# ugadiarov-la-phystech-edu/OCRL

Measured on AMD Instinct MI355X. Metric: images/sec (node) SLATE pretrain 128x128, 6 slots, 3 iters, higher is better.
Workload: dtype f32

## Files before the change

ocrl_amd/_lib.py:

```python
import ctypes
import os
from ctypes import c_void_p

from . import _abi

_HERE = os.path.dirname(os.path.abspath(__file__))
LIB_PATH = os.environ.get("OCRL_HIP_LIB") or os.path.join(_HERE, "libocrl_hip.so")
HEADER_PATH = os.path.join(_HERE, os.pardir, "include", "ocrl_hip.h")
DQN_HEADER_PATH = os.path.join(_HERE, os.pardir, "include", "ocrl_hip_dqn.h")
ROLLOUT_HEADER_PATH = os.path.join(_HERE, os.pardir, "include", "ocrl_hip_rollout.h")
REPLAY_HEADER_PATH = os.path.join(_HERE, os.pardir, "include", "ocrl_hip_replay.h")
C51_HEADER_PATH = os.path.join(_HERE, os.pardir, "include", "ocrl_hip_c51.h")
_lib = None

if not os.path.exists(HEADER_PATH):
    raise RuntimeError(f"{HEADER_PATH} is missing: ocrl_amd derives its binding of libocrl_hip.so from the header and runs from the source tree.")
with open(HEADER_PATH) as _f:
    ABI = _abi.read(_f.read())
CONSTANTS = ABI.consts
SlateConfig, IodineConfig, GemmDesc, ConvDesc, ConvWgradDesc, XattnDesc, AcnetDesc, SpriteEnvDesc, ScenesDesc, FlatSegment = (
    ABI.structs["ocrl_" + n] for n in ("slate_config", "iodine_config", "gemm_desc", "conv_desc", "conv_wgrad_desc", "xattn_desc", "acnet_desc",
                                       "sprite_env_desc", "scenes_desc", "flat_segment"))
FLAT_MAX_SEGMENTS = CONSTANTS["OCRL_FLAT_MAX_SEGMENTS"]
if not os.path.exists(DQN_HEADER_PATH):
    raise RuntimeError(f"{DQN_HEADER_PATH} is missing: ocrl_amd derives its binding of libocrl_hip.so from the header and runs from the source tree.")
with open(DQN_HEADER_PATH) as _f:
    ABI_DQN = _abi.read(_f.read())
QnetDesc = ABI_DQN.structs["ocrl_qnet_desc"]
QNET_MAX_LAYERS = len(QnetDesc().dims)
if not os.path.exists(ROLLOUT_HEADER_PATH):
    raise RuntimeError(f"{ROLLOUT_HEADER_PATH} is missing: ocrl_amd derives its binding of libocrl_hip.so from the header and runs from the source tree.")
with open(ROLLOUT_HEADER_PATH) as _f:
    ABI_ROLLOUT = _abi.read(_f.read())
if not os.path.exists(REPLAY_HEADER_PATH):
    raise RuntimeError(f"{REPLAY_HEADER_PATH} is missing: ocrl_amd derives its binding of libocrl_hip.so from the header and runs from the source tree.")
with open(REPLAY_HEADER_PATH) as _f:
    ABI_REPLAY = _abi.read(_f.read())
if not os.path.exists(C51_HEADER_PATH):
    raise RuntimeError(f"{C51_HEADER_PATH} is missing: ocrl_amd derives its binding of libocrl_hip.so from the header and runs from the source tree.")
with open(C51_HEADER_PATH) as _f:
    ABI_C51 = _abi.read(_f.read())
C51Desc = ABI_C51.structs["ocrl_c51_desc"]


def flat_segments(segs):
    addr = lambda a: a.value if isinstance(a, c_void_p) else a
    return (FlatSegment * len(segs))(*[FlatSegment(addr(p), addr(g), addr(s0), addr(s1), int(n)) for p, g, s0, s1, n in segs])


def acnet_desc(B, F, A, dims, acts):
    d = AcnetDesc(B=B, F=F, A=A)
    for t in range(3):
        if len(dims[t]) > CONSTANTS["OCRL_ACNET_MAX_LAYERS"]:
            raise ValueError(f"ocrl_amd: at most {CONSTANTS['OCRL_ACNET_MAX_LAYERS']} layers per trunk (got {len(dims[t])})")
        d.n[t] = len(dims[t])
        for l, (w, a) in enumerate(zip(dims[t], acts[t])):
            d.dims[t][l], d.acts[t][l] = int(w), int(a)
    return d


def qnet_desc(B, F, A, dims, acts):
    if len(dims) > QNET_MAX_LAYERS or len(acts) != len(dims):
        raise ValueError(f"ocrl_amd: at most {QNET_MAX_LAYERS} hidden layers, one activation code each (got {len(dims)}, {len(acts)})")
    d = QnetDesc(B=B, F=F, A=A, n=len(dims))
    for l, (w, a) in enumerate(zip(dims, acts)):
# ... 21 lines not shown
    d = ConvDesc()
    for k, v in kw.items():
        setattr(d, k, v)
    return d


def conv_wgrad_desc(**kw):
    d = ConvWgradDesc()
    for k, v in kw.items():
        setattr(d, k, v)
    return d


def lib():
    global _lib
    if _lib is not None:
        return _lib
    if not os.path.exists(LIB_PATH):
        raise RuntimeError(
            f"{LIB_PATH} is missing: build it with `python -c 'import __graft_entry__ as g; g.build()'` "
            "(make -C ocrl_amd/csrc).  ocrl_amd has no CPU fallback.")
    import torch
    L = ctypes.CDLL(LIB_PATH)
    for abi in (ABI, ABI_DQN, ABI_ROLLOUT, ABI_REPLAY, ABI_C51):
        for name, (restype, argtypes) in abi.functions.items():
            f = getattr(L, name)
            f.argtypes = argtypes
            if restype is not ctypes.c_int:
                f.restype = restype
    for name, cls in {**ABI.structs, **ABI_DQN.structs, **ABI_C51.structs}.items():
        if name + "_size" in {**ABI.functions, **ABI_DQN.functions, **ABI_C51.functions} and getattr(L, name + "_size")() != ctypes.sizeof(cls):
            raise RuntimeError(f"libocrl_hip.so: {name} is {getattr(L, name + '_size')()} bytes, this binding's {cls.__name__} {ctypes.sizeof(cls)}")
    if L.ocrl_abi_version() != CONSTANTS["OCRL_ABI_VERSION"]:
        raise RuntimeError(f"libocrl_hip.so ABI version mismatch: the library is {L.ocrl_abi_version()}, include/ocrl_hip.h {CONSTANTS['OCRL_ABI_VERSION']}")
    _lib = L
    return L


def check(rc):
    if rc:
        raise RuntimeError("ocrl_hip: " + lib().ocrl_last_error().decode())


def ptr(t):
    return None if t is None else ctypes.c_void_p(t.data_ptr())


# ... 8 lines not shown
```

ocrl_amd/csrc/kernels.h:

```cpp
#pragma once
#include "common.h"
#include "../../include/ocrl_hip.h"

enum { PROF_CONV5 = 0, PROF_CONV_OTHER = 1, PROF_WGRAD = 2, PROF_GEMM = 3, PROF_SA_FWD = 4, PROF_SA_BWD = 5, PROF_ATTN_FWD = 6, PROF_ATTN_BWD = 7, PROF_NTAGS = 8 };
int prof_begin(int tag, hipStream_t st);
void prof_end(int idx, hipStream_t st);

struct GemmArgs {
    const float* A = nullptr;
    const float* B = nullptr;
    float* C = nullptr;
    int M = 0, N = 0, K = 0;
    int lda = 0, ldb = 0, ldc = 0;
    int akc = 1, bkc = 1;
    int batch = 1;
    int batch_inner = 1;
    long long sA = 0, sB = 0, sC = 0;
    long long sAi = 0, sBi = 0, sCi = 0;
    int splitk = 1;
    long long sCsplit = 0;
    float alpha = 1.f;
    const float* bias = nullptr;
    int relu = 0;
    float drop_p = 0.f;
// ... 190 lines not shown
    int B = 0, H = 0, W = 0;
    float* bpart = nullptr;
};
int conv_fwd_launch(const ConvArgs& a, int KS, int CIN, int COUT, hipStream_t st, int low_latency = 0);
int conv_wgrad_launch(const WgradArgs& a, int KS, int CIN, int COUT, int cin_real, float* dW, float* db, int accumulate, hipStream_t st, int x3 = -1);
int conv_wgrad_slabs(int B, int H, int W, int KS, int CIN);
size_t conv_wgrad_ws_floats(int B, int H, int W, int KS, int CIN, bool with_db = true);
int conv_pack_launch(const float* W, float* fwd, float* bwd, int KS, int CIN, int COUT, int cin_real, hipStream_t st);

size_t conv_first_pack_floats();
int conv_first_pack_launch(const float* W, float* pack, hipStream_t st);
int conv_first_fwd_launch(const float* obs, const float* pack, const float* bias, float* Y, int B, int H, int W, int relu, hipStream_t st);
int conv_first_wgrad_workers(int B, int H, int W);
size_t conv_first_wgrad_ws_floats(int B, int H, int W);
int conv_first_wgrad_launch(const float* obs, const float* dY, float* ws, float* dW, float* db, int B, int H, int W, int accumulate, hipStream_t st);

int nchw_to_nhwc8_launch(const float* in, float* out, int B, int C, int H, int W, hipStream_t st);
int patchify4_launch(const float* in, float* out, int B, int C, int S, hipStream_t st);
int pixel_shuffle_launch(const float* in, float* out, int B, int h, int w, int Cout, int forward, const float* mask, hipStream_t st);
int layernorm_fwd_launch(const float* x, const float* g, const float* b, float* y, float* mean, float* rstd, long long R, int F, hipStream_t st);
int layernorm_bwd_launch(const float* dy, const float* x, const float* mean, const float* rstd, const float* g, float* dx,
                         float* dgb, long long R, int F, int accumulate_dx, int accumulate_dgb, float* ws, size_t ws_floats, hipStream_t st);
int colsum_launch(const float* X, long long ld, float* out, long long R, int F, int accumulate, float scale, float* ws, size_t ws_floats, hipStream_t st);

#define SA_INPUT_SLAB (2 * 4096 + 4 * 64)
void sa_input_plan(long long R, int max_wgs, int out[3]);
int sa_input_fwd_launch(const float* e4, const float* gamma, const float* beta, const float* W0, const float* b0, const float* W2, const float* b2,
                        float* mean, float* rstd, float* ln0, float* h1, float* x, long long R, int max_wgs, hipStream_t st);
int sa_input_bwd_launch(const float* dx, const float* h1, const float* e4, const float* mean, const float* rstd, const float* gamma, const float* beta,
                        const float* W0, const float* W2, float* de4, float* dW0, float* db0, float* dW2, float* db2, float* dgamma, float* dbeta,
                        long long R, int max_wgs, float* ws, size_t ws_floats, hipStream_t st);
int reduce_partials_launch(const float* part, int n, float* out, float scale, int accumulate, hipStream_t st);
int mse_launch(const float* obs, const float* recon, float* drecon, float* out, int B, int C, int H, int W, float* ws, size_t ws_floats, hipStream_t st);
int gumbel_softmax_launch(const float* raw, const float* e1, const float* e2, float* z, int* tokens, long long R, int V, float tau,
                          unsigned long long seed, hipStream_t st, float* zst = nullptr);
int softmax_bwd_rows_launch(const float* z, float* d, long long R, int V, float scale, hipStream_t st);
int softmax_stat_combine_launch(const float* stat, int nseg, long long R, float* lse, const float* hstat, const int* hidx, int* tokens,
                                const float* pred, int ldp, const int* tok, float* out, float scale, float* ws, size_t ws_floats, hipStream_t st,
                                const float* cdf_scores = nullptr, int cdf_V = 0, float cdf_tau = 1.f, unsigned long long cdf_seed = 0);
int exp_rows_launch(const float* y, const float* lse, float* z, long long R, int V, hipStream_t st);
int rowdot_bias64_launch(const float* g, const float* act, const float* bias, long long R, float* out, hipStream_t st);
int embed_fwd_launch(const int* tokens, const float* dict, const float* bos, const float* pe, float* out, int B, int T, int d, float p,
                     unsigned long long seed, hipStream_t st);
size_t embed_bwd_ws_floats(long long BT, int V, int d);
int embed_bwd_launch(float* g, const int* tokens, float* ddict, int B, int T, int V, int d, float p, unsigned long long seed, float* ws,
                     size_t ws_floats, hipStream_t st);
// ... 211 lines not shown
```

ocrl_amd/csrc/slate_model.cpp:

```cpp
#include "slate_model.h"

#include "switches.h"

#include <math.h>
#include <stdarg.h>
#include <string.h>

static std::string fmt(const char* f, ...) {
    char buf[256];
    va_list ap;
    va_start(ap, f);
    vsnprintf(buf, sizeof buf, f, ap);
    va_end(ap);
    return buf;
}

SlateModel::SlateModel(const SlateConfig& c) : cfg(c) {
    S = c.obs_size; E = S / 4; T = E * E; N = S * S; V = c.vocab; d = c.d_model; C = c.cnn_hidden;
    K = c.num_slots; I = c.num_iters; D = c.slot_size; H = c.mlp_hidden; NB = c.num_blocks; NH = c.num_heads;
    DH = d / NH; Bmax = c.max_batch; SH = c.slot_heads > 0 ? c.slot_heads : 1;
    const int ch = c.obs_channels;
    add_param("_dvae._encoder.0.m.weight", {64, ch, 4, 4}, 0); add_param("_dvae._encoder.0.m.bias", {64}, 0);
    for (int i = 1; i < 7; ++i) { add_param(fmt("_dvae._encoder.%d.m.weight", i), {64, 64, 1, 1}, 0); add_param(fmt("_dvae._encoder.%d.m.bias", i), {64}, 0); }
    add_param("_dvae._encoder.7.weight", {V, 64, 1, 1}, 0); add_param("_dvae._encoder.7.bias", {V}, 0);
// ... 165 lines not shown
                if (ws_commit_) { x3_of_[bc_pk_[i]] = f3; x3_of_[bc_pkb_[i]] = b3; }
            }
        }
        bc_Wk4_ = carve(nullptr, 9 * 64 * 4); bc_Wb4_ = carve(nullptr, 9 * 64 * 4);
        bc_dW1r_ = carve(nullptr, (size_t)25 * 64 * D); bc_dWc_ = carve(nullptr, 25 * 64 * 5 + 64);
        bc_dT_ = carve(nullptr, BK * 1600); bc_dM_ = carve(nullptr, BK * 1600); bc_G1_ = carve(nullptr, (size_t)N * 64);
        recon_ = carve("recon", BN * 4);
    } else {
    patches_ = carve("patches", BT * 16 * cfg.obs_channels);
    for (int i = 0; i < 7; ++i) de_[i] = carve(fmt("dvae_enc%d", i).c_str(), BT * 64);
    zraw_ = carve("zraw", BT * V);
    z_ = carve("z", BT * V);
    zdec_ = cfg.hard ? carve("z_st", BT * V) : z_;
    tokens_ = reinterpret_cast<int*>(carve("tokens", BT));
    {
        const size_t nseg = (size_t)gemm_stat_segments(V);
        zstat_ = carve(nullptr, BT * nseg * 2); zhstat_ = carve(nullptr, BT * nseg); zhidx_ = reinterpret_cast<int*>(carve(nullptr, BT * nseg));
        zlse_ = carve("z_lse", BT); zdot_ = carve(nullptr, BT);
        cestat_ = carve(nullptr, BT * nseg * 2); celse_ = carve("ce_lse", BT); cepart_ = carve(nullptr, BT / 16 + 16);
    }
    dd0_ = carve("dvae_dec0", BT * 64); dd1_ = carve("dvae_dec1", BT * 64); dd2_ = carve("dvae_dec2", BT * 64); dd3_ = carve("dvae_dec3", BT * 64);
    dd4_ = carve("dvae_dec4", BT * 256); ps1_ = carve(nullptr, BT * 256);
    dd6_ = carve("dvae_dec6", BT * 256); dd7_ = carve("dvae_dec7", BT * 256); dd8_ = carve("dvae_dec8", BT * 256);
    dd9_ = carve("dvae_dec9", BT * 1024); ps2_ = carve(nullptr, BN * 64);
    recon_ = carve("recon", BN * 4); drecon_ = carve(nullptr, BN * 4);
    for (int i = 0; i < 2; ++i) {
        dw_fwd_[i] = carve(nullptr, 9 * 64 * 64); dw_bwd_[i] = carve(nullptr, 9 * 64 * 64);
        if (conv_x3_ > 0) {
            float* f3 = carve(nullptr, conv_x3_pack_floats(3));
            float* b3 = carve(nullptr, conv_x3_pack_floats(3));
            if (ws_commit_) { x3_of_[dw_fwd_[i]] = f3; x3_of_[dw_bwd_[i]] = b3; }
        }
    }
    w11p_ = carve(nullptr, 4 * 64);
    mem_ = carve("mem", BK * d); emb_ = carve("emb", BT * d);
    for (int b = 0; b < NB; ++b) {
        Blk& k = blk_[b];
        k.ln1 = carve(nullptr, BT * d); k.ln1_mean = carve(nullptr, BT); k.ln1_rstd = carve(nullptr, BT);
        k.q = carve(nullptr, BT * 3 * d); k.k = k.q + d; k.v = k.q + 2 * d;
        k.lse = carve(nullptr, B * NH * (size_t)T); k.ao = carve(nullptr, BT * d); k.x1 = carve(nullptr, BT * d);
        k.ln2 = carve(nullptr, BT * d); k.ln2_mean = carve(nullptr, BT); k.ln2_rstd = carve(nullptr, BT);
        k.cq = carve(nullptr, BT * d); k.ck = carve(nullptr, BK * d); k.cv = carve(nullptr, BK * d);
        k.cP = carve(nullptr, B * NH * (size_t)T * K); k.cao = carve(nullptr, BT * d); k.x2 = carve(nullptr, BT * d);
        k.ln3 = carve(nullptr, BT * d); k.ln3_mean = carve(nullptr, BT); k.ln3_rstd = carve(nullptr, BT);
        k.f1 = carve(fmt("blk%d.ffn_hidden", b).c_str(), BT * 4 * d); k.x3 = carve(nullptr, BT * d);
    }
    bg_.resize(NB);
    {
        const size_t NC = xattn_supported(K, d, NH) ? (size_t)NH * xattn_kp(K, NH) : 16;
        xa_zero_base_ = carve_pos();
        for (int b = 0; b < NB; ++b) {
            Blk& k = blk_[b];
            k.xaAb = carve(nullptr, B * NC * d); k.xaAbT = carve(nullptr, B * NC * d); k.xaVo = carve(nullptr, B * NC * d); k.xaVoT = carve(nullptr, B * NC * d);
        }
        xa_zero_floats_ = (size_t)(carve_pos() - xa_zero_base_);
        for (int b = 0; b < NB; ++b) { bg_[b].xaPd = carve(nullptr, BT * NC); bg_[b].xaDs = carve(nullptr, BT * NC); }
        xa_dAb_ = carve(nullptr, B * NC * d); xa_dVo_ = carve(nullptr, B * NC * d);
// ... 93 lines not shown
}

int SlateModel::pack_weights(const Lane& L, bool encoder_only) {
    if (first_direct()) RC(conv_first_pack_launch(P(w_.enc[0].w), cw_fwd_[0], L));
    else RC(conv_pack_launch(P(w_.enc[0].w), cw_fwd_[0], nullptr, 5, 8, 64, cfg.obs_channels, L));
    RC(conv_pack_launch(P(w_.enc[1].w), cw_fwd_[1], cw_bwd_[1], 5, 64, 64, 64, L));
    RC(conv_pack_launch(P(w_.enc[2].w), cw_fwd_[2], cw_bwd_[2], 5, 64, 64, 64, L));
    RC(conv_pack_launch(P(w_.enc[3].w), cw_fwd_[3], cw_bwd_[3], 5, 64, 64, 64, L));
    if (conv_x3_ > 0) {
        for (int i = 1; i < 4; ++i) {
            auto f = x3_of_.find(cw_fwd_[i]), b = x3_of_.find(cw_bwd_[i]);
            if (f != x3_of_.end()) RC(conv_pack_x3_launch(P(w_.enc[i].w), const_cast<float*>(f->second), b != x3_of_.end() ? const_cast<float*>(b->second) : nullptr, L));
        }
    }
    if (!cfg.use_bcdec && !encoder_only) {
        RC(conv_pack_launch(P(w_.dvae_dec[1].w), dw_fwd_[0], dw_bwd_[0], 3, 64, 64, 64, L));
        RC(conv_pack_launch(P(w_.dvae_dec[6].w), dw_fwd_[1], dw_bwd_[1], 3, 64, 64, 64, L));
        if (conv_x3_ > 0) {
            for (int i = 0; i < 2; ++i) {
                auto f = x3_of_.find(dw_fwd_[i]), b = x3_of_.find(dw_bwd_[i]);
                if (f != x3_of_.end()) RC(conv_pack_x3_launch(P(w_.dvae_dec[i ? 6 : 1].w), const_cast<float*>(f->second), b != x3_of_.end() ? const_cast<float*>(b->second) : nullptr, L, 3));
            }
        }
        RC(copy_launch(P(w_.dvae_dec[11].w), w11p_, cfg.obs_channels * 64, L));
        RC(fill_launch(w11p_ + cfg.obs_channels * 64, (4 - cfg.obs_channels) * 64, 0.f, L));
    }
    RC(pack_launch(sa_pack_dev_, sa_pack_n_, sa_pack_max_, sa_wts_, L));
    RC(posmap_launch(P(w_.enc_pos.w), P(w_.enc_pos.b), posmap_, S, C, L));
    return 0;
}

int SlateModel::fwd_encoder(const StepInputs& in, const Lane& L, FwdDvae fork) {
    const int B = in.B;
    const long long BN = (long long)B * N;
    auto fork_if = [&](FwdDvae here) -> int {
        if (fork != here) return 0;
        RC(after(dvae_lane(), L, ev_fork_));
        return fwd_dvae(in, dvae_lane());
    };
    RC(slot_init_launch(P(w_.sa.mu), P(w_.sa.log_sigma), in.noise_slots, slots0_, B * K, D, in.seed, L, in.seed_dev));
    SlotAttnArgs a = sa_args(B, N, K, D, H, I, SH);
    a.x = x_; a.slots0 = slots0_; a.wts = sa_wts_; a.slots = slots_; a.attn = attn_; a.attn_heads = attn_heads_; a.save = sa_save_;
    if (conv_lowlat_ && frozen_) a.save = nullptr;
    a.xchg = sa_xchg_; a.parts = sa_parts_;
    a.phase = 1;
    RC(slot_attn_launch(a, 0, L));
    RC(fork_if(FwdDvae::AtStart));
    if (first_direct()) {
// ... 51 lines not shown
}

int SlateModel::dvae_decode(int B, float* drecon, const Lane& L, const float* zin) {
    const long long BT = (long long)B * T, BN = (long long)B * N;
    const int ch = cfg.obs_channels;
    if (!zin && fused_heads()) {
        GemmArgs a;
        a.A = zraw_; a.B = P(w_.dvae_dec[0].w); a.C = dd0_; a.M = (int)BT; a.N = 64; a.K = V; a.lda = V; a.ldb = V; a.ldc = 64;
        a.bias = P(w_.dvae_dec[0].b); a.relu = 1; a.a_mode = 2; a.x_lse = zlse_;
        RC(gemm_launch(a, L));
    } else {
    if (!zin) zin = zdec_;
    RC(lin_fwd(zin, V, P(w_.dvae_dec[0].w), P(w_.dvae_dec[0].b), dd0_, 64, BT, 64, V, 1, nullptr, 0, 0.f, 0, L));
    }
    RC(conv_layer_fwd(dd0_, dw_fwd_[0], P(w_.dvae_dec[1].b), dd1_, B, E, E, 3, 64, 1, nullptr, nullptr, L));
    RC(lin_fwd(dd1_, 64, P(w_.dvae_dec[2].w), P(w_.dvae_dec[2].b), dd2_, 64, BT, 64, 64, 1, nullptr, 0, 0.f, 0, L));
    RC(lin_fwd(dd2_, 64, P(w_.dvae_dec[3].w), P(w_.dvae_dec[3].b), dd3_, 64, BT, 64, 64, 1, nullptr, 0, 0.f, 0, L));
    RC(lin_fwd(dd3_, 64, P(w_.dvae_dec[4].w), P(w_.dvae_dec[4].b), dd4_, 256, BT, 256, 64, 1, nullptr, 0, 0.f, 0, L));
    RC(pixel_shuffle_launch(dd4_, ps1_, B, E, E, 64, 1, nullptr, L));
    RC(conv_layer_fwd(ps1_, dw_fwd_[1], P(w_.dvae_dec[6].b), dd6_, B, 2 * E, 2 * E, 3, 64, 1, nullptr, nullptr, L));
    RC(lin_fwd(dd6_, 64, P(w_.dvae_dec[7].w), P(w_.dvae_dec[7].b), dd7_, 64, 4 * BT, 64, 64, 1, nullptr, 0, 0.f, 0, L));
    RC(lin_fwd(dd7_, 64, P(w_.dvae_dec[8].w), P(w_.dvae_dec[8].b), dd8_, 64, 4 * BT, 64, 64, 1, nullptr, 0, 0.f, 0, L));
    RC(lin_fwd(dd8_, 64, P(w_.dvae_dec[9].w), P(w_.dvae_dec[9].b), dd9_, 256, 4 * BT, 256, 64, 1, nullptr, 0, 0.f, 0, L));
    RC(pixel_shuffle_launch(dd9_, ps2_, B, 2 * E, 2 * E, 64, 1, nullptr, L));
    RC(lin_fwd(ps2_, 64, P(w_.dvae_dec[11].w), P(w_.dvae_dec[11].b), recon_, 4, BN, ch, 64, 0, nullptr, 0, 0.f, 0, L));
    RC(mse_launch(last_.obs, recon_, drecon, metrics_ + (drecon ? 0 : 4), B, ch, S, S, L.scratch, L.scratch_floats, L));
    return 0;
}

AttnArgs SlateModel::self_attn_args(int b) const {
    const Blk& k = blk_[b];
    AttnArgs a;
    a.q = k.q; a.k = k.k; a.v = k.v; a.o = k.ao; a.lse = k.lse; a.B = last_.B; a.T = T; a.d = d; a.h = NH; a.ld = 3 * d;
    a.p = pdrop_; a.seed = last_.seed; a.site = SITE_BLK_BASE + 8 * b + 0;
    return a;
}
XaHost SlateModel::xattn_args(int b) const {
    const Blk& k = blk_[b];
    const unsigned site = SITE_BLK_BASE + 8 * b;
    XaHost hx;
    hx.x = k.ln2; hx.P = k.cP; hx.Ab = k.xaAb; hx.AbT = k.xaAbT; hx.Vo = k.xaVo; hx.VoT = k.xaVoT;
    hx.B = last_.B; hx.T = T; hx.K = K; hx.d = d; hx.h = NH; hx.p = pdrop_; hx.seed = last_.seed; hx.site_p = site + 2; hx.site_o = site + 3;
    return hx;
}

int SlateModel::fwd_decoder(const Lane& L, bool with_ce) {
    const int B = last_.B;
    const long long BT = (long long)B * T;
// ... 349 lines not shown
    RC(colsum_launch(gmap_, C, G(w_.enc[3].b), N, C, 0, 1.f, L.scratch, L.scratch_floats, L));
    RC(conv_layer_wgrad(e3_, gB_, G(w_.enc[3].w), nullptr, B, S, S, 5, 64, 64, L));
    RC(conv_layer_fwd(gB_, cw_bwd_[3], nullptr, gA_, B, S, S, 5, 64, 0, nullptr, e3_, L));
    RC(conv_layer_wgrad(e2_, gA_, G(w_.enc[2].w), G(w_.enc[2].b), B, S, S, 5, 64, 64, L));
    RC(conv_layer_fwd(gA_, cw_bwd_[2], nullptr, gB_, B, S, S, 5, 64, 0, nullptr, e2_, L));
    RC(conv_layer_wgrad(e1_, gB_, G(w_.enc[1].w), G(w_.enc[1].b), B, S, S, 5, 64, 64, L));
    RC(conv_layer_fwd(gB_, cw_bwd_[1], nullptr, gA_, B, S, S, 5, 64, 0, nullptr, e1_, L));
    if (first_direct()) {
        OCRL_REQUIRE(conv_first_wgrad_ws_floats(B, S, S) <= L.scratch_floats, "first conv wgrad: scratch too small");
        RC(conv_first_wgrad_launch(obs_keep_, gA_, L.scratch, G(w_.enc[0].w), G(w_.enc[0].b), B, S, S, 0, L));
    } else {
        const int ch = cfg.obs_channels, ldc0 = (25 * ch + 3) & ~3;
        if (!side_w) RC(im2col5_launch(obs8_, col0_, BN, S, S, ch, ldc0, L));
        RC(lin_bwd_w(gA_, 64, col0_, ldc0, dw0p_, G(w_.enc[0].b), BN, 64, ldc0, 1.f, L));
        RC(unpack5_launch(dw0p_, G(w_.enc[0].w), ch, ldc0, L));
    }
    return 0;
}

int SlateModel::bwd_dvae(const Lane& L) {
    const int B = last_.B;
    const long long BT = (long long)B * T, BN = (long long)B * N;
    const int ch = cfg.obs_channels;
    float* w4 = L.scratch + L.scratch_floats - 1024;
    {
        GemmArgs a;
        a.A = drecon_; a.B = ps2_; a.C = w4; a.M = 4; a.N = 64; a.K = (int)BN; a.lda = 4; a.ldb = 64; a.ldc = 64; a.akc = 0; a.bkc = 0;
        long long splits = BN / 512; if (splits > 512) splits = 512; if (splits < 1) splits = 1;
        if (splits > 1) {
            a.splitk = (int)splits; a.C = L.scratch; a.sCsplit = 256;
            RC(gemm_launch(a, L));
            RC(splitk_reduce_launch(L.scratch, w4, 256, (int)splits, 256, 0, L));
        } else RC(gemm_launch(a, L));
        RC(copy_launch(w4, G(w_.dvae_dec[11].w), ch * 64, L));
        RC(colsum_launch(drecon_, 4, w4 + 256, BN, 4, 0, 1.f, L.scratch, L.scratch_floats - 1024, L));
        RC(copy_launch(w4 + 256, G(w_.dvae_dec[11].b), ch, L));
    }
    RC(lin_bwd_x(drecon_, 4, w11p_, gdA_, 64, BN, 4, 64, nullptr, 0, nullptr, 0, L));
    RC(pixel_shuffle_launch(gdA_, gdB_, B, 2 * E, 2 * E, 64, 0, dd9_, L));
    RC(lin_bwd_w(gdB_, 256, dd8_, 64, G(w_.dvae_dec[9].w), G(w_.dvae_dec[9].b), 4 * BT, 256, 64, 1.f, L));
    RC(lin_bwd_x(gdB_, 256, P(w_.dvae_dec[9].w), gdA_, 64, 4 * BT, 256, 64, dd8_, 64, nullptr, 0, L));
    RC(lin_bwd_w(gdA_, 64, dd7_, 64, G(w_.dvae_dec[8].w), G(w_.dvae_dec[8].b), 4 * BT, 64, 64, 1.f, L));
    RC(lin_bwd_x(gdA_, 64, P(w_.dvae_dec[8].w), gdB_, 64, 4 * BT, 64, 64, dd7_, 64, nullptr, 0, L));
    RC(lin_bwd_w(gdB_, 64, dd6_, 64, G(w_.dvae_dec[7].w), G(w_.dvae_dec[7].b), 4 * BT, 64, 64, 1.f, L));
    RC(lin_bwd_x(gdB_, 64, P(w_.dvae_dec[7].w), gdA_, 64, 4 * BT, 64, 64, dd6_, 64, nullptr, 0, L));
    RC(conv_layer_wgrad(ps1_, gdA_, G(w_.dvae_dec[6].w), G(w_.dvae_dec[6].b), B, 2 * E, 2 * E, 3, 64, 64, L));
    RC(conv_layer_fwd(gdA_, dw_bwd_[1], nullptr, gdB_, B, 2 * E, 2 * E, 3, 64, 0, nullptr, ps1_, L));
    RC(pixel_shuffle_launch(gdB_, gdA_, B, E, E, 64, 0, nullptr, L));
    RC(lin_bwd_w(gdA_, 256, dd3_, 64, G(w_.dvae_dec[4].w), G(w_.dvae_dec[4].b), BT, 256, 64, 1.f, L));
    RC(lin_bwd_x(gdA_, 256, P(w_.dvae_dec[4].w), gdB_, 64, BT, 256, 64, dd3_, 64, nullptr, 0, L));
    RC(lin_bwd_w(gdB_, 64, dd2_, 64, G(w_.dvae_dec[3].w), G(w_.dvae_dec[3].b), BT, 64, 64, 1.f, L));
    RC(lin_bwd_x(gdB_, 64, P(w_.dvae_dec[3].w), gdA_, 64, BT, 64, 64, dd2_, 64, nullptr, 0, L));
    RC(lin_bwd_w(gdA_, 64, dd1_, 64, G(w_.dvae_dec[2].w), G(w_.dvae_dec[2].b), BT, 64, 64, 1.f, L));
    RC(lin_bwd_x(gdA_, 64, P(w_.dvae_dec[2].w), gdB_, 64, BT, 64, 64, dd1_, 64, nullptr, 0, L));
    RC(conv_layer_wgrad(dd0_, gdB_, G(w_.dvae_dec[1].w), G(w_.dvae_dec[1].b), B, E, E, 3, 64, 64, L));
    RC(conv_layer_fwd(gdB_, dw_bwd_[0], nullptr, gdA_, B, E, E, 3, 64, 0, nullptr, dd0_, L));
    float* dz = zraw_;
    have_scores_ = false;
    if (fused_heads()) {
        Xf zx; zx.b_mode = 2; zx.lse = zlse_;
        RC(lin_bwd_w(gdA_, 64, zraw_, V, G(w_.dvae_dec[0].w), G(w_.dvae_dec[0].b), BT, 64, V, 1.f, L, zx));
        RC(rowdot_bias64_launch(gdA_, dd0_, P(w_.dvae_dec[0].b), BT, zdot_, L));
// ... 128 lines not shown
```

ocrl_amd/csrc/slate_model.h:

```cpp
#pragma once
#include <map>
#include <string>
#include <vector>

#include "kernels.h"
#include "model_base.h"
#include "slot_attn_host.h"
#include "stream_plan.h"

struct SlateConfig {
    int obs_size = 64, obs_channels = 3, vocab = 4096, d_model = 192, cnn_hidden = 64;
    int num_slots = 5, num_iters = 3, slot_size = 192, mlp_hidden = 192;
    int num_blocks = 4, num_heads = 4;
    float dropout = 0.1f;
    int max_batch = 1;
    int use_bcdec = 0;
    int hard = 0;
    int slot_heads = 1;
};

struct StepInputs {
    const float* obs = nullptr;
    int B = 0;
    float tau = 1.f;
// ... 87 lines not shown
    long long group_begin_[4] = {0, 0, 0, 0};

    int S, E, T, N, V, d, C, K, I, D, H, NB, NH, DH, Bmax;
    int SH = 1;
    StepInputs last_;
    float pdrop_ = 0.f;
    bool have_fwd_ = false;
    int conv_lowlat_ = 0;
    bool frozen_ = false, packs_valid_ = false;
    bool have_enc_ = false;
    bool enc_only_grads_ = false;
    bool have_scores_ = false;

    float *scratch_ = nullptr;
    size_t scratch_floats_ = 0;
    float* scratch2_ = nullptr;
    StreamPlan plan_;
    hipStream_t side_ = nullptr;
    hipEvent_t ev_fork_ = nullptr, ev_join_ = nullptr, ev_tokens_ = nullptr;
    float *zstat_ = nullptr, *zhstat_ = nullptr, *zlse_ = nullptr, *zdot_ = nullptr, *cestat_ = nullptr, *celse_ = nullptr, *cepart_ = nullptr;
    int* zhidx_ = nullptr;
    float *obs8_, *patches_, *de_[7], *zraw_, *z_, *zdec_;
    int* tokens_;
    float *dd0_, *dd1_, *dd2_, *dd3_, *dd4_, *ps1_, *dd6_, *dd7_, *dd8_, *dd9_, *ps2_, *recon_, *drecon_;
    float *e1_, *e2_, *e3_, *e4_, *posmap_, *gridT_, *ln0_, *ln0_mean_, *ln0_rstd_, *h1_, *x_;
    float *slots0_, *slot_noise_, *slots_, *attn_, *sa_save_, *sa_wts_, *sa_grows_, *sa_small_, *sa_xchg_;
    float* attn_heads_ = nullptr;
    float* sa_parts_;
    PackEntry* sa_pack_dev_ = nullptr;
    int sa_pack_n_ = 0, sa_pack_max_ = 0;
    float *cw_fwd_[4], *cw_bwd_[4];
    int conv_x3_ = 0;
    std::map<const float*, const float*> x3_of_;
    float *dw_fwd_[2], *dw_bwd_[2];
    float *w11p_;
    float *mem_, *emb_;
    struct Blk {
        float *ln1, *ln1_mean, *ln1_rstd, *q, *k, *v, *lse, *ao, *x1;
        float *ln2, *ln2_mean, *ln2_rstd, *cq, *ck, *cv, *cP, *cao, *x2;
        float *ln3, *ln3_mean, *ln3_rstd, *f1, *x3;
        float *xaAb, *xaAbT, *xaVo, *xaVoT;
    };
    int sa_input_ = 1;
    bool xattn_ = false;
    float *xa_dAb_ = nullptr, *xa_dVo_ = nullptr, *xa_pq_ = nullptr, *xa_po_ = nullptr;
    size_t xa_zero_floats_ = 0;
    float* xa_zero_base_ = nullptr;
    std::vector<Blk> blk_;
    struct BlkG { float *gbr[3], *gf1, *gt2, *gqkv, *xaPd, *xaDs; };
    std::vector<BlkG> bg_;
    struct EncGraph { hipGraphExec_t exec = nullptr; int warm = 0; };
    std::map<int, EncGraph> enc_graphs_;
    int enc_graph_mode_ = -1;
    hipStream_t cap_ = nullptr;
    float* obs_stage_ = nullptr;
    unsigned long long* seed_dev_ = nullptr;
    hipStream_t side2_ = nullptr;
    float* scratch3_ = nullptr;
// ... 19 lines not shown
```

Measured before the change: 1796.

## Fuse dVAE decoder pixel-shuffle into final 1x1 conv head fwd/bwd kernels

Replaces the pixel_shuffle plus GEMM for the last dVAE decoder layer with dedicated kernels that read dd9 directly in its pre-shuffle layout. Forward, the input gradient with ReLU mask, and the weight gradient each get their own kernel, which removes the ps2 intermediate buffer, the padded weight copy and the separate shuffle pass. The aim is to cut memory traffic over the full-resolution tensor and the number of launches. In exchange it adds hand-written kernels whose strided gather in the weight-gradient path may be less efficient than the generic GEMM.

```diff
diff --git a/include/ocrl_hip_dvae_head.h b/include/ocrl_hip_dvae_head.h
--- /dev/null
+++ b/include/ocrl_hip_dvae_head.h
@@ -0,0 +1,17 @@
+#ifndef OCRL_HIP_DVAE_HEAD_H
+#define OCRL_HIP_DVAE_HEAD_H
+#include <stddef.h>
+
+#ifdef __cplusplus
+extern "C" {
+#endif
+
+size_t ocrl_dvae_head_ws_floats(int B, int S);
+int ocrl_dvae_head_fwd(const float* dd9, const float* w, const float* bias, float* recon, int B, int S, int C, void* stream);
+int ocrl_dvae_head_bwd(const float* dd9, const float* drecon, const float* w, float* ddd9 , float* dw ,
+                       int B, int S, int C, float* ws, size_t ws_floats, void* stream);
+
+#ifdef __cplusplus
+}
+#endif
+#endif
diff --git a/ocrl_amd/_lib.py b/ocrl_amd/_lib.py
--- a/ocrl_amd/_lib.py
+++ b/ocrl_amd/_lib.py
@@ -11,6 +11,7 @@
 ROLLOUT_HEADER_PATH = os.path.join(_HERE, os.pardir, "include", "ocrl_hip_rollout.h")
 REPLAY_HEADER_PATH = os.path.join(_HERE, os.pardir, "include", "ocrl_hip_replay.h")
 C51_HEADER_PATH = os.path.join(_HERE, os.pardir, "include", "ocrl_hip_c51.h")
+DVAE_HEAD_HEADER_PATH = os.path.join(_HERE, os.pardir, "include", "ocrl_hip_dvae_head.h")
 _lib = None
 
 if not os.path.exists(HEADER_PATH):
@@ -41,6 +42,10 @@
 with open(C51_HEADER_PATH) as _f:
     ABI_C51 = _abi.read(_f.read())
 C51Desc = ABI_C51.structs["ocrl_c51_desc"]
+if not os.path.exists(DVAE_HEAD_HEADER_PATH):
+    raise RuntimeError(f"{DVAE_HEAD_HEADER_PATH} is missing: ocrl_amd derives its binding of libocrl_hip.so from the header and runs from the source tree.")
+with open(DVAE_HEAD_HEADER_PATH) as _f:
+    ABI_DVAE_HEAD = _abi.read(_f.read())
 
 
 def flat_segments(segs):
@@ -108,7 +113,7 @@
             "(make -C ocrl_amd/csrc).  ocrl_amd has no CPU fallback.")
     import torch
     L = ctypes.CDLL(LIB_PATH)
-    for abi in (ABI, ABI_DQN, ABI_ROLLOUT, ABI_REPLAY, ABI_C51):
+    for abi in (ABI, ABI_DQN, ABI_ROLLOUT, ABI_REPLAY, ABI_C51, ABI_DVAE_HEAD):
         for name, (restype, argtypes) in abi.functions.items():
             f = getattr(L, name)
             f.argtypes = argtypes
diff --git a/ocrl_amd/csrc/dvae_head.hip b/ocrl_amd/csrc/dvae_head.hip
--- /dev/null
+++ b/ocrl_amd/csrc/dvae_head.hip
@@ -0,0 +1,256 @@
+#include "common.h"
+#include "kernels.h"
+
+namespace {
+constexpr int FWD_ROWS = 64;
+constexpr int FWD_LD = 128 + 4;
+constexpr int DW_TP = 64;
+
+__device__ __forceinline__ constexpr int k_of(int n) { return (n >> 1) + 4 * (n & 1); }
+
+__global__ __launch_bounds__(256, 4) void dvae_head_fwd_kernel(const float* __restrict__ dd9, const float* __restrict__ W, const float* __restrict__ bias,
+                                                            float* __restrict__ recon, long long R, int W2, int S, int ch) {
+    __shared__ __attribute__((aligned(16))) float sx[FWD_ROWS * FWD_LD];
+    __shared__ float4 sw[64];
+    const int t = threadIdx.x;
+    if (t < 64) {
+        float4 w = make_float4(0.f, 0.f, 0.f, 0.f);
+        w.x = W[t];
+        if (ch > 1) w.y = W[64 + t];
+        if (ch > 2) w.z = W[128 + t];
+        if (ch > 3) w.w = W[192 + t];
+        sw[t] = w;
+    }
+    const float b0 = bias[0], b1 = ch > 1 ? bias[1] : 0.f, b2 = ch > 2 ? bias[2] : 0.f, b3 = ch > 3 ? bias[3] : 0.f;
+    const int c4 = t & 31, r0 = t >> 5;
+    const int lr = (t >> 6) * 16 + ((t & 63) >> 2), sub = t & 3;
+    const long long npass = (R + FWD_ROWS - 1) / FWD_ROWS;
+    for (long long pass = blockIdx.x; pass < npass; pass += gridDim.x) {
+        const long long row0 = pass * FWD_ROWS;
+        float4 v[2][FWD_ROWS / 8];
+#pragma unroll
+        for (int half = 0; half < 2; ++half)
+#pragma unroll
+            for (int n = 0; n < FWD_ROWS / 8; ++n) {
+                const long long row = row0 + r0 + 8 * n;
+                v[half][n] = row < R ? *reinterpret_cast<const float4*>(dd9 + (size_t)row * 256 + half * 128 + c4 * 4) : make_float4(0.f, 0.f, 0.f, 0.f);
+            }
+        const float* xr = sx + lr * FWD_LD + sub;
+        float a0 = 0.f, a1 = 0.f, a2 = 0.f, a3 = 0.f;
+#pragma unroll
+        for (int half = 0; half < 2; ++half) {
+            __syncthreads();
+#pragma unroll
+            for (int n = 0; n < FWD_ROWS / 8; ++n) *reinterpret_cast<float4*>(sx + (r0 + 8 * n) * FWD_LD + c4 * 4) = v[half][n];
+            __syncthreads();
+#pragma unroll 1
+            for (int c8 = 0; c8 < 4; ++c8) {
+#pragma unroll
+                for (int n = 0; n < 8; ++n) {
+                    const int c = c8 * 8 + k_of(n);
+                    const float x = xr[4 * c];
+                    const float4 w = sw[half * 32 + c];
+                    a0 = __builtin_fmaf(x, w.x, a0); a1 = __builtin_fmaf(x, w.y, a1); a2 = __builtin_fmaf(x, w.z, a2); a3 = __builtin_fmaf(x, w.w, a3);
+                }
+            }
+        }
+        const long long row = row0 + lr;
+        if (row < R) {
+            const long long bh = row / W2;
+            const int w = (int)(row - bh * W2);
+            const long long pix = (2 * bh + (sub >> 1)) * S + 2 * w + (sub & 1);
+            float4 o = make_float4(a0 + b0, 0.f, 0.f, 0.f);
+            if (ch > 1) o.y = a1 + b1;
+            if (ch > 2) o.z = a2 + b2;
+            if (ch > 3) o.w = a3 + b3;
+            *reinterpret_cast<float4*>(recon + pix * 4) = o;
+        }
+    }
+}
+
+__global__ __launch_bounds__(256) void dvae_head_dx_kernel(const float* __restrict__ drecon, const float* __restrict__ W, const float* __restrict__ dd9,
+                                                           float* __restrict__ gd, long long R, int W2, int S, int ch) {
+    const int c = threadIdx.x & 63;
+    float w[4];
+#pragma unroll
+    for (int k = 0; k < 4; ++k) w[k] = k < ch ? W[k * 64 + c] : 0.f;
+    const long long nw = (long long)gridDim.x * 4;
+    const int wv = __builtin_amdgcn_readfirstlane(threadIdx.x >> 6);
+#pragma unroll 2
+    for (long long row = (long long)blockIdx.x * 4 + wv; row < R; row += nw) {
+        const long long bh = row / W2;
+        const int x2 = (int)(row - bh * W2);
+        const float4 m = *reinterpret_cast<const float4*>(dd9 + (size_t)row * 256 + c * 4);
+        const float* d0 = drecon + ((2 * bh) * S + 2 * x2) * 4;
+        const float* d1 = d0 + (size_t)S * 4;
+        const float4 p00 = *reinterpret_cast<const float4*>(d0), p01 = *reinterpret_cast<const float4*>(d0 + 4);
+        const float4 p10 = *reinterpret_cast<const float4*>(d1), p11 = *reinterpret_cast<const float4*>(d1 + 4);
+        const float pk[4][4] = {{p00.x, p00.y, p00.z, p00.w}, {p01.x, p01.y, p01.z, p01.w}, {p10.x, p10.y, p10.z, p10.w}, {p11.x, p11.y, p11.z, p11.w}};
+        float a[4] = {0.f, 0.f, 0.f, 0.f};
+#pragma unroll
+        for (int k = 0; k < 4; ++k)
+            if (k < ch) {
+#pragma unroll
+                for (int s = 0; s < 4; ++s) a[s] = __builtin_fmaf(pk[s][k], w[k], a[s]);
+            }
+        float4 o;
+        o.x = m.x > 0.f ? a[0] : 0.f; o.y = m.y > 0.f ? a[1] : 0.f; o.z = m.z > 0.f ? a[2] : 0.f; o.w = m.w > 0.f ? a[3] : 0.f;
+        *reinterpret_cast<float4*>(gd + (size_t)row * 256 + c * 4) = o;
+    }
+}
+
+__global__ __launch_bounds__(256) void dvae_head_dw_kernel(const float* __restrict__ drecon, const float* __restrict__ dd9, float* __restrict__ part,
+                                                           long long BN, int S, int kt_per, int ch) {
+    __shared__ float sx[2][DW_TP][64];
+    __shared__ __attribute__((aligned(16))) float sd[2][4][DW_TP];
+    __shared__ int so[2][DW_TP];
+    const int t = threadIdx.x, k = t >> 6, c = t & 63;
+    const long long p0 = (long long)blockIdx.x * kt_per * 32;
+    long long p1 = p0 + (long long)kt_per * 32;
+    if (p1 > BN) p1 = BN;
+    const int nst = p1 > p0 ? (int)((p1 - p0 + DW_TP - 1) / DW_TP) : 0;
+    const int W2 = S >> 1;
+    auto offsets = [&](int st) {
+        if (t < DW_TP) {
+            const long long p = p0 + (long long)st * DW_TP + t;
+            int o = -1;
+            if (p < p1) {
+                const long long by = p / S;
+                const int x = (int)(p - by * S);
+                const long long row = (by >> 1) * W2 + (x >> 1);
+                o = (int)(row * 4 + 2 * (by & 1) + (x & 1));
+            }
+            so[st & 1][t] = o;
+        }
+    };
+    float xv[DW_TP / 4];
+    float4 dv = make_float4(0.f, 0.f, 0.f, 0.f);
+    auto load = [&](int st) {
+#pragma unroll
+        for (int n = 0; n < DW_TP / 4; ++n) {
+            const int o = so[st & 1][k + 4 * n];
+            xv[n] = o >= 0 ? dd9[(size_t)(o >> 2) * 256 + 4 * c + (o & 3)] : 0.f;
+        }
+        if (t < DW_TP) {
+            const long long p = p0 + (long long)st * DW_TP + t;
+            dv = p < p1 ? *reinterpret_cast<const float4*>(drecon + p * 4) : make_float4(0.f, 0.f, 0.f, 0.f);
+        }
+    };
+    auto store = [&](int st) {
+#pragma unroll
+        for (int n = 0; n < DW_TP / 4; ++n) sx[st & 1][k + 4 * n][c] = xv[n];
+        if (t < DW_TP) { sd[st & 1][0][t] = dv.x; sd[st & 1][1][t] = dv.y; sd[st & 1][2][t] = dv.z; sd[st & 1][3][t] = dv.w; }
+    };
+    float acc = 0.f;
+    if (nst > 0) {
+        offsets(0);
+        offsets(1);
+        __syncthreads();
+        load(0);
+        store(0);
+    }
+    for (int st = 0; st < nst; ++st) {
+        __syncthreads();
+        if (st + 1 < nst) load(st + 1);
+        if (st + 2 < nst) offsets(st + 2);
+        if (k < ch) {
+            const float(*x)[64] = sx[st & 1];
+            const float* d = sd[st & 1][k];
+#pragma unroll
+            for (int q8 = 0; q8 < DW_TP; q8 += 8) {
+                const float4 da = *reinterpret_cast<const float4*>(d + q8), db = *reinterpret_cast<const float4*>(d + q8 + 4);
+                acc = __builtin_fmaf(da.x, x[q8 + 0][c], acc); acc = __builtin_fmaf(db.x, x[q8 + 4][c], acc);
+                acc = __builtin_fmaf(da.y, x[q8 + 1][c], acc); acc = __builtin_fmaf(db.y, x[q8 + 5][c], acc);
+                acc = __builtin_fmaf(da.z, x[q8 + 2][c], acc); acc = __builtin_fmaf(db.z, x[q8 + 6][c], acc);
+                acc = __builtin_fmaf(da.w, x[q8 + 3][c], acc); acc = __builtin_fmaf(db.w, x[q8 + 7][c], acc);
+            }
+        }
+        if (st + 1 < nst) store(st + 1);
+    }
+    if (k < ch) part[(size_t)blockIdx.x * 256 + t] = acc;
+}
+
+__global__ __launch_bounds__(256) void dvae_head_dw_reduce_kernel(const float* __restrict__ part, float* __restrict__ out, int n, int splits) {
+    __shared__ float red[16][16];
+    const int cl = threadIdx.x & 15, sl = threadIdx.x >> 4;
+    const int e = blockIdx.x * 16 + cl;
+    float s = 0.f;
+    if (e < n) {
+        int k = sl;
+        for (; k + 48 < splits; k += 64) {
+            const float v0 = part[(size_t)k * 256 + e], v1 = part[(size_t)(k + 16) * 256 + e];
+            const float v2 = part[(size_t)(k + 32) * 256 + e], v3 = part[(size_t)(k + 48) * 256 + e];
+            s += (v0 + v1) + (v2 + v3);
+        }
+        for (; k < splits; k += 16) s += part[(size_t)k * 256 + e];
+    }
+    red[sl][cl] = s;
+    __syncthreads();
+    if (sl == 0 && e < n) {
+        float r = 0.f;
+#pragma unroll
+        for (int k = 0; k < 16; ++k) r += red[k][cl];
+        out[e] = r;
+    }
+}
+
+}
+
+int dvae_head_check(const char* who, int B, int S, int ch) {
+    OCRL_REQUIRE(B >= 1 && S >= 2 && S % 2 == 0, "%s: batch >= 1 and an even image size >= 2 (got %d, %d)", who, B, S);
+    OCRL_REQUIRE(ch >= 1 && ch <= 4, "%s: 1 <= channels <= 4 (got %d)", who, ch);
+    OCRL_REQUIRE((long long)B * S * S < (1LL << 29), "%s: %d images of %d x %d leave the int32 range of one call", who, B, S, S);
+    return 0;
+}
+
+int dvae_head_fwd_launch(const float* dd9, const float* W, const float* b, float* recon, int B, int S, int ch, hipStream_t st) {
+    RC(dvae_head_check("dvae_head_fwd", B, S, ch));
+    OCRL_REQUIRE(((((uintptr_t)dd9) | ((uintptr_t)recon)) & 15) == 0, "dvae_head_fwd: dd9 and recon must be 16-byte aligned");
+    const long long R = (long long)B * (S / 2) * (S / 2);
+    long long grid = (R + FWD_ROWS - 1) / FWD_ROWS;
+    if (grid > 1024) grid = 1024;
+    hipLaunchKernelGGL(dvae_head_fwd_kernel, dim3((unsigned)grid), dim3(256), 0, st, dd9, W, b, recon, R, S / 2, S, ch);
+    OCRL_CHECK_LAUNCH("dvae_head_fwd");
+    return 0;
+}
+
+int dvae_head_dx_launch(const float* drecon, const float* W, const float* dd9, float* gd, int B, int S, int ch, hipStream_t st) {
+    RC(dvae_head_check("dvae_head_dx", B, S, ch));
+    OCRL_REQUIRE(((((uintptr_t)dd9) | ((uintptr_t)drecon) | ((uintptr_t)gd)) & 15) == 0, "dvae_head_dx: dd9, drecon and the gradient must be 16-byte aligned");
+    const long long R = (long long)B * (S / 2) * (S / 2);
+    long long grid = (R + 3) / 4;
+    if (grid > 2048) grid = 2048;
+    hipLaunchKernelGGL(dvae_head_dx_kernel, dim3((unsigned)grid), dim3(256), 0, st, drecon, W, dd9, gd, R, S / 2, S, ch);
+    OCRL_CHECK_LAUNCH("dvae_head_dx");
+    return 0;
+}
+
+int dvae_head_dw_splits(long long BN) {
+    long long s = BN / 512;
+    if (s > 512) s = 512;
+    return s < 1 ? 1 : (int)s;
+}
+size_t dvae_head_dw_ws_floats(long long BN) {
+    const int s = dvae_head_dw_splits(BN);
+    return s > 1 ? (size_t)s * 256 : 0;
+}
+
+int dvae_head_dw_launch(const float* drecon, const float* dd9, float* dW, int B, int S, int ch, float* ws, size_t ws_floats, hipStream_t st) {
+    RC(dvae_head_check("dvae_head_dw", B, S, ch));
+    OCRL_REQUIRE((((uintptr_t)drecon) & 15) == 0, "dvae_head_dw: drecon must be 16-byte aligned");
+    const long long BN = (long long)B * S * S;
+    const int splits = dvae_head_dw_splits(BN);
+    const int nkt = (int)((BN + 31) / 32), kt_per = (nkt + splits - 1) / splits;
+    if (splits == 1) {
+        hipLaunchKernelGGL(dvae_head_dw_kernel, dim3(1), dim3(256), 0, st, drecon, dd9, dW, BN, S, kt_per, ch);
+        OCRL_CHECK_LAUNCH("dvae_head_dw");
+        return 0;
+    }
+    OCRL_REQUIRE(ws && ws_floats >= dvae_head_dw_ws_floats(BN), "dvae_head_dw: workspace too small (%zu < %zu floats)", ws ? ws_floats : (size_t)0,
+                 dvae_head_dw_ws_floats(BN));
+    hipLaunchKernelGGL(dvae_head_dw_kernel, dim3(splits), dim3(256), 0, st, drecon, dd9, ws, BN, S, kt_per, ch);
+    OCRL_CHECK_LAUNCH("dvae_head_dw");
+    hipLaunchKernelGGL(dvae_head_dw_reduce_kernel, dim3(cdiv(ch * 64, 16)), dim3(256), 0, st, ws, dW, ch * 64, splits);
+    OCRL_CHECK_LAUNCH("dvae_head_dw_reduce");
+    return 0;
+}
diff --git a/ocrl_amd/csrc/dvae_head_unit.cpp b/ocrl_amd/csrc/dvae_head_unit.cpp
--- /dev/null
+++ b/ocrl_amd/csrc/dvae_head_unit.cpp
@@ -0,0 +1,32 @@
+#include "../../include/ocrl_hip_dvae_head.h"
+#include "common.h"
+#include "kernels.h"
+
+extern "C" {
+
+size_t ocrl_dvae_head_ws_floats(int B, int S) {
+    if (dvae_head_check("ocrl_dvae_head_ws_floats", B, S, 1)) return 0;
+    return dvae_head_dw_ws_floats((long long)B * S * S);
+}
+
+int ocrl_dvae_head_fwd(const float* dd9, const float* w, const float* bias, float* recon, int B, int S, int C, void* stream) {
+    RC(dvae_head_check("ocrl_dvae_head_fwd", B, S, C));
+    OCRL_REQUIRE(dd9 && w && bias && recon, "ocrl_dvae_head_fwd: null argument");
+    return dvae_head_fwd_launch(dd9, w, bias, recon, B, S, C, static_cast<hipStream_t>(stream));
+}
+
+int ocrl_dvae_head_bwd(const float* dd9, const float* drecon, const float* w, float* ddd9, float* dw, int B, int S, int C, float* ws, size_t ws_floats,
+                       void* stream) {
+    RC(dvae_head_check("ocrl_dvae_head_bwd", B, S, C));
+    OCRL_REQUIRE(dd9 && drecon && w, "ocrl_dvae_head_bwd: null argument");
+    OCRL_REQUIRE(ddd9 || dw, "ocrl_dvae_head_bwd: ddd9 and dw are both null: nothing to write");
+    OCRL_REQUIRE(((((uintptr_t)dd9) | ((uintptr_t)drecon) | ((uintptr_t)ddd9)) & 15) == 0, "ocrl_dvae_head_bwd: dd9, drecon and ddd9 must be 16-byte aligned");
+    const size_t need = dvae_head_dw_ws_floats((long long)B * S * S);
+    if (dw) OCRL_REQUIRE(need == 0 || (ws && ws_floats >= need), "ocrl_dvae_head_bwd: workspace too small (%zu < %zu floats)", ws ? ws_floats : (size_t)0, need);
+    hipStream_t st = static_cast<hipStream_t>(stream);
+    if (dw) RC(dvae_head_dw_launch(drecon, dd9, dw, B, S, C, ws, ws_floats, st));
+    if (ddd9) RC(dvae_head_dx_launch(drecon, w, dd9, ddd9, B, S, C, st));
+    return 0;
+}
+
+}
diff --git a/ocrl_amd/csrc/kernels.h b/ocrl_amd/csrc/kernels.h
--- a/ocrl_amd/csrc/kernels.h
+++ b/ocrl_amd/csrc/kernels.h
@@ -236,6 +236,13 @@
 int layernorm_bwd_launch(const float* dy, const float* x, const float* mean, const float* rstd, const float* g, float* dx,
                          float* dgb, long long R, int F, int accumulate_dx, int accumulate_dgb, float* ws, size_t ws_floats, hipStream_t st);
 int colsum_launch(const float* X, long long ld, float* out, long long R, int F, int accumulate, float scale, float* ws, size_t ws_floats, hipStream_t st);
+
+int dvae_head_check(const char* who, int B, int S, int ch);
+int dvae_head_fwd_launch(const float* dd9, const float* W, const float* b, float* recon, int B, int S, int ch, hipStream_t st);
+int dvae_head_dx_launch(const float* drecon, const float* W, const float* dd9, float* gd, int B, int S, int ch, hipStream_t st);
+int dvae_head_dw_splits(long long BN);
+size_t dvae_head_dw_ws_floats(long long BN);
+int dvae_head_dw_launch(const float* drecon, const float* dd9, float* dW, int B, int S, int ch, float* ws, size_t ws_floats, hipStream_t st);
 
 #define SA_INPUT_SLAB (2 * 4096 + 4 * 64)
 void sa_input_plan(long long R, int max_wgs, int out[3]);
diff --git a/ocrl_amd/csrc/slate_model.cpp b/ocrl_amd/csrc/slate_model.cpp
--- a/ocrl_amd/csrc/slate_model.cpp
+++ b/ocrl_amd/csrc/slate_model.cpp
@@ -211,7 +211,7 @@
     dd0_ = carve("dvae_dec0", BT * 64); dd1_ = carve("dvae_dec1", BT * 64); dd2_ = carve("dvae_dec2", BT * 64); dd3_ = carve("dvae_dec3", BT * 64);
     dd4_ = carve("dvae_dec4", BT * 256); ps1_ = carve(nullptr, BT * 256);
     dd6_ = carve("dvae_dec6", BT * 256); dd7_ = carve("dvae_dec7", BT * 256); dd8_ = carve("dvae_dec8", BT * 256);
-    dd9_ = carve("dvae_dec9", BT * 1024); ps2_ = carve(nullptr, BN * 64);
+    dd9_ = carve("dvae_dec9", BT * 1024);
     recon_ = carve("recon", BN * 4); drecon_ = carve(nullptr, BN * 4);
     for (int i = 0; i < 2; ++i) {
         dw_fwd_[i] = carve(nullptr, 9 * 64 * 64); dw_bwd_[i] = carve(nullptr, 9 * 64 * 64);
@@ -221,7 +221,6 @@
             if (ws_commit_) { x3_of_[dw_fwd_[i]] = f3; x3_of_[dw_bwd_[i]] = b3; }
         }
     }
-    w11p_ = carve(nullptr, 4 * 64);
     mem_ = carve("mem", BK * d); emb_ = carve("emb", BT * d);
     for (int b = 0; b < NB; ++b) {
         Blk& k = blk_[b];
@@ -361,8 +360,6 @@
                 if (f != x3_of_.end()) RC(conv_pack_x3_launch(P(w_.dvae_dec[i ? 6 : 1].w), const_cast<float*>(f->second), b != x3_of_.end() ? const_cast<float*>(b->second) : nullptr, L, 3));
             }
         }
-        RC(copy_launch(P(w_.dvae_dec[11].w), w11p_, cfg.obs_channels * 64, L));
-        RC(fill_launch(w11p_ + cfg.obs_channels * 64, (4 - cfg.obs_channels) * 64, 0.f, L));
     }
     RC(pack_launch(sa_pack_dev_, sa_pack_n_, sa_pack_max_, sa_wts_, L));
     RC(posmap_launch(P(w_.enc_pos.w), P(w_.enc_pos.b), posmap_, S, C, L));
@@ -460,8 +457,7 @@
     RC(lin_fwd(dd6_, 64, P(w_.dvae_dec[7].w), P(w_.dvae_dec[7].b), dd7_, 64, 4 * BT, 64, 64, 1, nullptr, 0, 0.f, 0, L));
     RC(lin_fwd(dd7_, 64, P(w_.dvae_dec[8].w), P(w_.dvae_dec[8].b), dd8_, 64, 4 * BT, 64, 64, 1, nullptr, 0, 0.f, 0, L));
     RC(lin_fwd(dd8_, 64, P(w_.dvae_dec[9].w), P(w_.dvae_dec[9].b), dd9_, 256, 4 * BT, 256, 64, 1, nullptr, 0, 0.f, 0, L));
-    RC(pixel_shuffle_launch(dd9_, ps2_, B, 2 * E, 2 * E, 64, 1, nullptr, L));
-    RC(lin_fwd(ps2_, 64, P(w_.dvae_dec[11].w), P(w_.dvae_dec[11].b), recon_, 4, BN, ch, 64, 0, nullptr, 0, 0.f, 0, L));
+    RC(dvae_head_fwd_launch(dd9_, P(w_.dvae_dec[11].w), P(w_.dvae_dec[11].b), recon_, B, S, ch, L));
     RC(mse_launch(last_.obs, recon_, drecon, metrics_ + (drecon ? 0 : 4), B, ch, S, S, L.scratch, L.scratch_floats, L));
     return 0;
 }
@@ -857,22 +853,13 @@
     const int B = last_.B;
     const long long BT = (long long)B * T, BN = (long long)B * N;
     const int ch = cfg.obs_channels;
-    float* w4 = L.scratch + L.scratch_floats - 1024;
+    RC(dvae_head_dw_launch(drecon_, dd9_, G(w_.dvae_dec[11].w), B, S, ch, L.scratch, L.scratch_floats, L));
     {
-        GemmArgs a;
-        a.A = drecon_; a.B = ps2_; a.C = w4; a.M = 4; a.N = 64; a.K = (int)BN; a.lda = 4; a.ldb = 64; a.ldc = 64; a.akc = 0; a.bkc = 0;
-        long long splits = BN / 512; if (splits > 512) splits = 512; if (splits < 1) splits = 1;
-        if (splits > 1) {
-            a.splitk = (int)splits; a.C = L.scratch; a.sCsplit = 256;
-            RC(gemm_launch(a, L));
-            RC(splitk_reduce_launch(L.scratch, w4, 256, (int)splits, 256, 0, L));
-        } else RC(gemm_launch(a, L));
-        RC(copy_launch(w4, G(w_.dvae_dec[11].w), ch * 64, L));
-        RC(colsum_launch(drecon_, 4, w4 + 256, BN, 4, 0, 1.f, L.scratch, L.scratch_floats - 1024, L));
-        RC(copy_launch(w4 + 256, G(w_.dvae_dec[11].b), ch, L));
-    }
-    RC(lin_bwd_x(drecon_, 4, w11p_, gdA_, 64, BN, 4, 64, nullptr, 0, nullptr, 0, L));
-    RC(pixel_shuffle_launch(gdA_, gdB_, B, 2 * E, 2 * E, 64, 0, dd9_, L));
+        float* b4 = L.scratch + L.scratch_floats - 768;
+        RC(colsum_launch(drecon_, 4, b4, BN, 4, 0, 1.f, L.scratch, L.scratch_floats - 1024, L));
+        RC(copy_launch(b4, G(w_.dvae_dec[11].b), ch, L));
+    }
+    RC(dvae_head_dx_launch(drecon_, P(w_.dvae_dec[11].w), dd9_, gdB_, B, S, ch, L));
     RC(lin_bwd_w(gdB_, 256, dd8_, 64, G(w_.dvae_dec[9].w), G(w_.dvae_dec[9].b), 4 * BT, 256, 64, 1.f, L));
     RC(lin_bwd_x(gdB_, 256, P(w_.dvae_dec[9].w), gdA_, 64, 4 * BT, 256, 64, dd8_, 64, nullptr, 0, L));
     RC(lin_bwd_w(gdA_, 64, dd7_, 64, G(w_.dvae_dec[8].w), G(w_.dvae_dec[8].b), 4 * BT, 64, 64, 1.f, L));
diff --git a/ocrl_amd/csrc/slate_model.h b/ocrl_amd/csrc/slate_model.h
--- a/ocrl_amd/csrc/slate_model.h
+++ b/ocrl_amd/csrc/slate_model.h
@@ -133,7 +133,7 @@
     int* zhidx_ = nullptr;
     float *obs8_, *patches_, *de_[7], *zraw_, *z_, *zdec_;
     int* tokens_;
-    float *dd0_, *dd1_, *dd2_, *dd3_, *dd4_, *ps1_, *dd6_, *dd7_, *dd8_, *dd9_, *ps2_, *recon_, *drecon_;
+    float *dd0_, *dd1_, *dd2_, *dd3_, *dd4_, *ps1_, *dd6_, *dd7_, *dd8_, *dd9_, *recon_, *drecon_;
     float *e1_, *e2_, *e3_, *e4_, *posmap_, *gridT_, *ln0_, *ln0_mean_, *ln0_rstd_, *h1_, *x_;
     float *slots0_, *slot_noise_, *slots_, *attn_, *sa_save_, *sa_wts_, *sa_grows_, *sa_small_, *sa_xchg_;
     float* attn_heads_ = nullptr;
@@ -144,7 +144,6 @@
     int conv_x3_ = 0;
     std::map<const float*, const float*> x3_of_;
     float *dw_fwd_[2], *dw_bwd_[2];
-    float *w11p_;
     float *mem_, *emb_;
     struct Blk {
         float *ln1, *ln1_mean, *ln1_rstd, *q, *k, *v, *lse, *ao, *x1;
```

New measurement: 1813 (median of 6 runs). No clear change (+0.9%).
